# SqueezeAILab/SqueezeLLM

Hardware: AMD Instinct MI355X
Metric: LLaMA-7B-shaped quantised-linear decode throughput (batch 1, all QuantLinearLUT matvecs of the model per token) (higher is better)
Workload: dtype f32; 1 GPU; llama-7b w4 s0 (dense-only), batch=1 decode, 32 layers x 7 linears, op vecquant4matmul_nuq_perchannel; config_name=7b-w4-s0, launch=graph, linears sharing an input (q/k/v, gate/up) fused into one launch each, parallelism=single GPU, world_size=1, rccl_ranks=0

## Files before the change

### squeezellm_amd/csrc/sqllm_kernels.hip

```cpp
#include "sqllm_fused.h"
#include "sqllm_split_common.h"

namespace sqllm {

bool (*g_fused_variant)(int bits, const LaunchArgs& a, hipStream_t stream, hipError_t* err) = nullptr;

constexpr int kXtStride = 36;
constexpr int mfma_codebook_floats(int bits) { return bits == 4 ? 2 * 4096 / 4 : 4 * 8 * 128 / 4; }
constexpr int mfma_lds_floats(int bits, int mb, int waves) {
  return mfma_codebook_floats(bits) + cmax(waves * 16 * mb * kXtStride, waves * 16 * 64);
}

template <int BITS, int MB, int WAVES>
__device__ __forceinline__ void dense_role_mfma(const float* __restrict__ x, const u32x4* __restrict__ q,
                                                float* __restrict__ y, const float* __restrict__ lut, int K, int N,
                                                int batch, int m0, int bid, int n_col_tiles, int units_total,
                                                int units_per_wg, int units_stride, float* lds) {
  using F = Fmt<BITS>;
  constexpr int L = F::kLut, R = F::kRows, KU = F::kK;
  constexpr int NPH = KU / 8;
  constexpr int TR = 16 * MB;
  constexpr int XL = TR / 8;
  constexpr int ESTRIDE = (BITS == 4) ? 256 : 128;
  constexpr int SUBB = (BITS == 4) ? (L * ESTRIDE) / 2 : L * ESTRIDE;
  __builtin_amdgcn_s_waitcnt(0);
  const int tid = threadIdx.x;
  const int lane = tid & 63;
  const int wave = __builtin_amdgcn_readfirstlane(tid >> 6);
  const int i16 = lane & 15, grp = lane >> 4;
  if constexpr ((SQLLM_MFMA_VAR & 64) != 0) {
    const int pr = (wave >> 2) + ((SQLLM_MFMA_VAR & 128) ? 2 * ((bid >> 8) & 1) : 0);
    if (pr == 1) __builtin_amdgcn_s_setprio(1);
    else if (pr == 2) __builtin_amdgcn_s_setprio(2);
    else if (pr == 3) __builtin_amdgcn_s_setprio(3);
  }
  constexpr int kCb = mfma_codebook_floats(BITS);
  float* slabs = lds + kCb;
  float* xt = lds + kCb + wave * (TR * kXtStride);
  constexpr int EPW = 32 / WAVES, RPW = 16 / WAVES;
  constexpr int NE = (BITS == 4) ? EPW : RPW;
  const int st_j = (BITS == 4) ? 2 * (wave & 1) + (lane >> 5) : (wave & 3);
  const int st_h = (BITS == 4) ? (wave >> 1) : (wave >> 2);
  const int row_stride = N / 4;
  const char* qbase = reinterpret_cast<const char*>(q);
  const uint32_t row_bytes = 16u * (uint32_t)row_stride;
  int xrow[XL];
#pragma unroll
  for (int j = 0; j < XL; ++j) {
    int r = m0 + (lane >> 3) + 8 * j;
    if (r > batch - 1) r = batch - 1;
    xrow[j] = r * K + 4 * (lane & 1);
  }
  const int xkq = (lane >> 1) & 3;
  const uint32_t lane_off = 4 * (i16 + 16 * (grp & 1));
  uint32_t tb[4];
#pragma unroll
  for (int j = 0; j < 4; ++j) tb[j] = j * SUBB + 4 * (i16 + 16 * (grp & 1));
  float* xt_w = xt + (lane >> 3) * kXtStride + 8 * xkq + 4 * (lane & 1);
  const float* xt_r = xt + i16 * kXtStride + 8 * grp;

  const unsigned total = (unsigned)n_col_tiles * (unsigned)units_stride;
  unsigned gpos = (unsigned)bid * (unsigned)units_per_wg;
  unsigned gend = gpos + (unsigned)units_per_wg;
  if (gend > total) gend = total;
  while (gpos < gend) {
  const int ct = (int)(gpos / (unsigned)units_stride);
  const int u_beg = (int)(gpos - (unsigned)ct * (unsigned)units_stride);
  if (u_beg >= units_total) { gpos = (unsigned)(ct + 1) * (unsigned)units_stride; continue; }
  int u_end = units_total;
  if ((unsigned)(u_end - u_beg) > gend - gpos) u_end = u_beg + (int)(gend - gpos);
  gpos += (unsigned)(u_end - u_beg);
  if (u_end == units_total) gpos = (unsigned)(ct + 1) * (unsigned)units_stride;
  const int col0 = ct * kTileN;

  float ev[NE];
  {
    int c = col0 + 4 * i16 + st_j;
    if (c > N - 1) c = N - 1;
    const float* src = lut + (size_t)c * L;
    if constexpr (BITS == 4) {
#pragma unroll
      for (int i = 0; i < EPW / 4; ++i) {
        const f32x4 t = *reinterpret_cast<const f32x4*>(src + st_h * EPW + 4 * i);
        ev[4 * i] = t.x; ev[4 * i + 1] = t.y; ev[4 * i + 2] = t.z; ev[4 * i + 3] = t.w;
      }
    } else {
#pragma unroll
      for (int i = 0; i < RPW; ++i) ev[i] = src[2 * (st_h * RPW + i) + (lane >> 5)];
    }
  }
  const int n_groups_wg = (u_end - u_beg + 3) / 4;
  const int n_g = n_groups_wg > wave ? (n_groups_wg - wave + WAVES - 1) / WAVES : 0;
  int cidx = col0 / 4 + i16;
  if (cidx > row_stride - 1) cidx = row_stride - 1;
  const uint32_t lane_bytes = 16u * (uint32_t)cidx;
  auto group_unit = [&](int g, int kq) {
    return u_beg + 4 * (wave + WAVES * g) + kq;
  };
  auto load_w = [&](int g, u32x4 (&dw)[R]) {
    int u = group_unit(g, grp);
    if (u > u_end - 1) u = u_end - 1;
    if (u < u_beg) u = u_beg;
    if (SQLLM_MFMA_VAR & 32) u = u_beg + grp;
    const uint32_t off = (uint32_t)(u * R) * row_bytes + lane_bytes;
#pragma unroll
    for (int r = 0; r < R; ++r) dw[r] = __builtin_nontemporal_load(reinterpret_cast<const u32x4*>(qbase + (off + r * row_bytes)));
  };
  auto load_x = [&](int g, int ph, f32x4 (&dx)[XL]) {
    int u = group_unit(g, xkq);
    if (u > u_end - 1) u = u_end - 1;
    if (u < u_beg) u = u_beg;
    if ((SQLLM_MFMA_VAR & 16) && g > 0) return;
#pragma unroll
    for (int j = 0; j < XL; ++j) dx[j] = *reinterpret_cast<const f32x4*>(x + xrow[j] + u * KU + 8 * ph);
  };
  u32x4 wa[R], wb[R];
  f32x4 xa[XL], xb[XL];
  load_w(0, wa);
  load_x(0, 0, xa);
  asm volatile("" ::: "memory");
  __builtin_amdgcn_sched_barrier(0);
  if constexpr (BITS == 4) {
    float* dst = lds + ((wave & 1) * 4096 + st_h * EPW * ESTRIDE) / 4 + lane;
#pragma unroll
    for (int i = 0; i < EPW; ++i) dst[i * (ESTRIDE / 4)] = ev[i];
  } else {
    float* dst = lds + (st_j * SUBB) / 4 + (lane >> 5) * (ESTRIDE / 4) + (lane & 31);
#pragma unroll
    for (int i = 0; i < RPW; ++i) dst[2 * (st_h * RPW + i) * (ESTRIDE / 4)] = ev[i];
  }
  f32x4 acc[MB][4];
#pragma unroll
  for (int mb = 0; mb < MB; ++mb)
#pragma unroll
    for (int j = 0; j < 4; ++j) acc[mb][j] = f32x4{0.f, 0.f, 0.f, 0.f};
  __syncthreads();

  auto phase = [&](const float (&v)[4][8], const f32x4 (&dx)[XL], int g) {
    const bool live = group_unit(g, xkq) < u_end;
#pragma unroll
    for (int j = 0; j < XL; ++j)
      if (!(SQLLM_MFMA_VAR & 8)) *reinterpret_cast<f32x4*>(xt_w + 8 * j * kXtStride) = live ? dx[j] : f32x4{0.f, 0.f, 0.f, 0.f};
    f32x4 alo[MB], ahi[MB];
#pragma unroll
    for (int mb = 0; mb < MB; ++mb) {
      if constexpr (SQLLM_MFMA_VAR & 8) {
        alo[mb] = dx[0];
        ahi[mb] = dx[XL - 1];
      } else {
        alo[mb] = *reinterpret_cast<const f32x4*>(xt_r + 16 * mb * kXtStride);
        ahi[mb] = *reinterpret_cast<const f32x4*>(xt_r + 16 * mb * kXtStride + 4);
      }
    }
    if (SQLLM_MFMA_VAR & 1) __builtin_amdgcn_s_setprio(1);
#pragma unroll
    for (int s2 = 0; s2 < 8; ++s2)
#pragma unroll
      for (int mb = 0; mb < MB; ++mb) {
        const float a = s2 < 4 ? alo[mb][s2 & 3] : ahi[mb][s2 & 3];
#pragma unroll
        for (int j = 0; j < 4; ++j) {
#if SQLLM_MFMA_FAKE
          acc[mb][j].x = __builtin_fmaf(a, v[j][s2], acc[mb][j].x);
#else
          acc[mb][j] = __builtin_amdgcn_mfma_f32_16x16x4f32(a, v[j][s2], acc[mb][j], 0, 0, 0);
#endif
        }
      }
    if (SQLLM_MFMA_VAR & 1) __builtin_amdgcn_s_setprio(0);
  };
  auto lookups = [&](const u32x4 (&t)[R], auto ph_tag, float (&v)[4][8]) {
    constexpr int PH = decltype(ph_tag)::value;
    if constexpr (SQLLM_MFMA_VAR & 4) {
#pragma unroll
      for (int j = 0; j < 4; ++j)
#pragma unroll
        for (int i = 0; i < 8; ++i) v[j][i] = __builtin_bit_cast(float, t[0].x ^ (uint32_t)(j * 8 + i));
      return;
    }
    if constexpr (BITS == 4) {
      const uint32_t w4[4] = {t[0].x, t[0].y, t[0].z, t[0].w};
#pragma unroll
      for (int j = 0; j < 4; ++j) {
        const uint32_t lo = w4[j] & 0x0F0F0F0Fu, hi = (w4[j] >> 4) & 0x0F0F0F0Fu;
        const int off = (j >> 1) * 4096 + (j & 1) * 128;
        v[j][0] = lds_read_f32(__builtin_amdgcn_perm(lo, lane_off, 0x0C0C0400u) + off);
        v[j][1] = lds_read_f32(__builtin_amdgcn_perm(hi, lane_off, 0x0C0C0400u) + off);
        v[j][2] = lds_read_f32(__builtin_amdgcn_perm(lo, lane_off, 0x0C0C0500u) + off);
        v[j][3] = lds_read_f32(__builtin_amdgcn_perm(hi, lane_off, 0x0C0C0500u) + off);
        v[j][4] = lds_read_f32(__builtin_amdgcn_perm(lo, lane_off, 0x0C0C0600u) + off);
        v[j][5] = lds_read_f32(__builtin_amdgcn_perm(hi, lane_off, 0x0C0C0600u) + off);
        v[j][6] = lds_read_f32(__builtin_amdgcn_perm(lo, lane_off, 0x0C0C0700u) + off);
        v[j][7] = lds_read_f32(__builtin_amdgcn_perm(hi, lane_off, 0x0C0C0700u) + off);
      }
    } else {
      const uint32_t t0[4] = {t[0].x, t[0].y, t[0].z, t[0].w};
      const uint32_t t1[4] = {t[1].x, t[1].y, t[1].z, t[1].w};
      const uint32_t t2[4] = {t[2].x, t[2].y, t[2].z, t[2].w};
#pragma unroll
      for (int j = 0; j < 4; ++j) {
        v[j][0] = lds_read_f32(tb[j] | field3_x128<8 * PH + 0>(t0[j], t1[j], t2[j]));
        v[j][1] = lds_read_f32(tb[j] | field3_x128<8 * PH + 1>(t0[j], t1[j], t2[j]));
        v[j][2] = lds_read_f32(tb[j] | field3_x128<8 * PH + 2>(t0[j], t1[j], t2[j]));
        v[j][3] = lds_read_f32(tb[j] | field3_x128<8 * PH + 3>(t0[j], t1[j], t2[j]));
        v[j][4] = lds_read_f32(tb[j] | field3_x128<8 * PH + 4>(t0[j], t1[j], t2[j]));
        v[j][5] = lds_read_f32(tb[j] | field3_x128<8 * PH + 5>(t0[j], t1[j], t2[j]));
        v[j][6] = lds_read_f32(tb[j] | field3_x128<8 * PH + 6>(t0[j], t1[j], t2[j]));
        v[j][7] = lds_read_f32(tb[j] | field3_x128<8 * PH + 7>(t0[j], t1[j], t2[j]));
      }
    }
  };
  using P0 = std::integral_constant<int, 0>;
  using P1 = std::integral_constant<int, 1>;
  using P2 = std::integral_constant<int, 2>;
  using P3 = std::integral_constant<int, 3>;
  auto decode_group = [&](int g, const u32x4 (&w)[R], f32x4 (&xcur)[XL], u32x4 (&wn)[R], f32x4 (&xn)[XL]) {
    load_w(g + 1, wn);
    float v[4][8];
    if constexpr (NPH == 1) {
      load_x(g + 1, 0, xn);
      if (!(SQLLM_MFMA_VAR & 2)) __builtin_amdgcn_sched_barrier(0);
      lookups(w, P0{}, v);
      phase(v, xcur, g);
    } else {
      f32x4 xo[XL];
      load_x(g, 1, xo);
      if (!(SQLLM_MFMA_VAR & 2)) __builtin_amdgcn_sched_barrier(0);
      lookups(w, P0{}, v);
      phase(v, xcur, g);
      load_x(g, 2, xcur);
      if (!(SQLLM_MFMA_VAR & 2)) __builtin_amdgcn_sched_barrier(0);
      lookups(w, P1{}, v);
      phase(v, xo, g);
      load_x(g, 3, xo);
      if (!(SQLLM_MFMA_VAR & 2)) __builtin_amdgcn_sched_barrier(0);
      lookups(w, P2{}, v);
      phase(v, xcur, g);
      load_x(g + 1, 0, xn);
      if (!(SQLLM_MFMA_VAR & 2)) __builtin_amdgcn_sched_barrier(0);
      lookups(w, P3{}, v);
      phase(v, xo, g);
    }
    if (!(SQLLM_MFMA_VAR & 2)) __builtin_amdgcn_sched_barrier(0);
  };
  for (int g = 0; g < n_g; g += 2) {
    decode_group(g, wa, xa, wb, xb);
    decode_group(g + 1, wb, xb, wa, xa);
  }

  __syncthreads();
  float* slab = slabs + wave * (16 * 64) + (4 * grp) * 64 + 4 * i16;
#pragma unroll
  for (int mb = 0; mb < MB; ++mb) {
    if (mb) __syncthreads();
    *reinterpret_cast<f32x4*>(slab + 0 * 64) = f32x4{acc[mb][0].x, acc[mb][1].x, acc[mb][2].x, acc[mb][3].x};
    *reinterpret_cast<f32x4*>(slab + 1 * 64) = f32x4{acc[mb][0].y, acc[mb][1].y, acc[mb][2].y, acc[mb][3].y};
    *reinterpret_cast<f32x4*>(slab + 2 * 64) = f32x4{acc[mb][0].z, acc[mb][1].z, acc[mb][2].z, acc[mb][3].z};
    *reinterpret_cast<f32x4*>(slab + 3 * 64) = f32x4{acc[mb][0].w, acc[mb][1].w, acc[mb][2].w, acc[mb][3].w};
    __syncthreads();
#pragma unroll
    for (int e = tid; e < 16 * 64; e += WAVES * 64) {
      const int r = m0 + 16 * mb + (e >> 6);
      const int col = col0 + (e & 63);
      float sum = 0.f;
#pragma unroll
      for (int w = 0; w < WAVES; ++w) sum += slabs[w * (16 * 64) + e];
      if (r < batch && col < N) acc_add(y + (size_t)r * N + col, sum);
    }
  }
  }
}

template <int BITS, int MB, int WAVES>
__global__ void __launch_bounds__(WAVES * 64, (BITS == 4 && MB <= 2 && !(SQLLM_MFMA_VAR & 256)) ? 4 : 1)
sqllm_fused_batched(const float* x, const GroupArgs ga) {
  __shared__ __attribute__((aligned(16))) float lds[mfma_lds_floats(BITS, MB, WAVES)];
  const Segment sg = ga.seg[0];
  asm volatile("" ::SQLLM_SEG_OPERANDS(sg), "s"(x));
  __builtin_amdgcn_sched_barrier(0);
  const KernelGeom& gm = sg.gm;
  const int m0 = blockIdx.y * 16 * MB;
  dense_role_mfma<BITS, MB, WAVES>(x, reinterpret_cast<const u32x4*>(sg.q), sg.y, sg.lut, gm.K, gm.N, gm.batch, m0,
                                   (int)blockIdx.x, gm.col_tiles, gm.units_total, gm.units_per_wg, units_stride_of(gm), lds);
}

template <int WAVES>
__global__ void __launch_bounds__(WAVES * 64)
sqllm_sparse_batched(const float* x, const GroupArgs ga, const float* xT, int Bp, int pass_rows) {
  constexpr int T = WAVES * 64;
  __shared__ __attribute__((aligned(16))) float lds[kWideSparseLdsFloats];
  const Segment sg = ga.seg[0];
  asm volatile("" ::SQLLM_SEG_OPERANDS(sg), "s"(x));
  __builtin_amdgcn_sched_barrier(0);
  const KernelGeom& gm = sg.gm;
  const int sp = blockIdx.x;
  const int m0 = blockIdx.y * pass_rows;
  int rows_here = gm.batch - m0;
  if (rows_here > pass_rows) rows_here = pass_rows;
  if (sp < gm.csr_blocks) {
    if (xT) {
      csr_role<T, 1, float, float, true>(x, sg.y, sg.rows, sg.cols, sg.vals, gm.nnz, gm.K, gm.N, m0, rows_here, sp, lds, nullptr, 0, xT, Bp, SQLLM_PROBE_PTR(sg));
    } else {
      constexpr int CBT = 32;
      for (int bb = 0; bb < rows_here; bb += CBT) {
        if (bb) __syncthreads();
        csr_role<T, CBT, float, float>(x, sg.y, sg.rows, sg.cols, sg.vals, gm.nnz, gm.K, gm.N, m0 + bb,
                                       rows_here - bb < CBT ? rows_here - bb : CBT, sp, lds, nullptr, 0);
      }
    }
  } else if (sp < gm.csr_blocks + gm.topx_blocks) {
    for (int bb = 0; bb < rows_here; bb += 64) {
      if (bb) __syncthreads();
      topx_role<T, float, float, false, NoGate, 8>(x, sg.y, sg.full_rows, sg.full_idx, gm.topX, gm.K, gm.N, m0 + bb, rows_here - bb < 64 ? rows_here - bb : 64,
                                 sp - gm.csr_blocks, lds);
    }
  }
}

typedef float f32x8 __attribute__((ext_vector_type(8)));
constexpr int cols_table_floats(int bits) { return bits == 4 ? 17 * 64 : 65 * 64 * 2; }
constexpr int cols_lds_floats(int bits, int bt, int waves) {
  return cmax(cols_table_floats(bits) + waves * bt * 64, cmax(2 * kCsrSpanMax, kTopxLds));
}
constexpr int cols_stage_k(int bt) { return bt * 8 <= 32 ? 8 : 4; }

__device__ __forceinline__ uint32_t field6_x512(uint32_t t0, uint32_t t1, uint32_t t2, int M) {
  const int bit = 6 * M, w = bit >> 5, o = bit & 31;
  const uint32_t lo = (w == 0) ? t0 : (w == 1) ? t1 : t2;
  uint32_t f;
  if (o <= 26) {
    if (o > 9) f = lo >> (o - 9);
    else if (o < 9) f = lo << (9 - o);
    else f = lo;
  } else {
    const uint32_t hi = (w == 0) ? t1 : t2;
    f = __builtin_amdgcn_alignbit(hi, lo, o) << 9;
  }
  return f & 0x7E00u;
}

typedef const __attribute__((address_space(4))) float* cfloatp;
typedef const __attribute__((address_space(4))) char* ccharp;
template <int ST> struct XVec;
template <> struct XVec<4> {
  typedef f32x4 type;
  static __device__ __forceinline__ type load(ccharp base, uint32_t off) {
    return *reinterpret_cast<const __attribute__((address_space(4))) type*>(base + off);
  }
};
template <> struct XVec<8> {
  typedef f32x8 type;
  static __device__ __forceinline__ type load(ccharp base, uint32_t off) {
    return *reinterpret_cast<const __attribute__((address_space(4))) type*>(base + off);
  }
};

template <int BITS, int BT, int WAVES>
__device__ __forceinline__ void dense_role_cols(const float* __restrict__ x, const uint32_t* __restrict__ q,
                                                float* __restrict__ y, const float* __restrict__ lut, int K, int N,
                                                int b0, int nb, int bid, int n_col_tiles, int units_total,
                                                int units_per_wg, int units_stride, float* lds) {
  using F = Fmt<BITS>;
  constexpr int L = F::kLut, R = F::kRows, KU = F::kK;
  constexpr int ST = cols_stage_k(BT);
  constexpr int SPU = KU / ST;
  constexpr int D = BITS == 4 ? 4 : 2;
  constexpr int NB = 2;
  constexpr int NS = D * SPU;
  constexpr int NP = ST / 2;
  constexpr int NA = BT >= 4 ? 1 : 4 / BT;
  using XV = typename XVec<ST>::type;
  static_assert(NS % 2 == 0, "stages alternate between two register sets");
  static_assert(WAVES == 8, "table build assumes 8 waves");
  __builtin_amdgcn_s_waitcnt(0);
  const int tid = threadIdx.x, lane = tid & 63;
  const int w = __builtin_amdgcn_readfirstlane(tid >> 6);
  char* table = reinterpret_cast<char*>(lds);
  float* slabs = lds + cols_table_floats(BITS);
  const uint32_t lane_base = BITS == 4 ? (4u * lane) | 0x1000u : 8u * lane;
  const uint32_t row_bytes = 4u * (uint32_t)N;
  ccharp xrow[BT];
#pragma unroll
  for (int b = 0; b < BT; ++b) xrow[b] = reinterpret_cast<ccharp>(reinterpret_cast<uintptr_t>(x + (size_t)(b0 + (b < nb ? b : nb - 1)) * K));
  uint32_t soff[D][R];
#pragma unroll
  for (int j = 0; j < D; ++j)
#pragma unroll
    for (int r = 0; r < R; ++r) soff[j][r] = (uint32_t)(j * WAVES * R + r) * row_bytes;
  if constexpr (BITS == 4) { if (tid < 64) *reinterpret_cast<float*>(table + 16 * 256 + 4 * tid) = 0.f; }
  else { if (tid < 64) *reinterpret_cast<f32x2*>(table + 64 * 512 + 8 * tid) = f32x2{0.f, 0.f}; }

  const unsigned total = (unsigned)n_col_tiles * (unsigned)units_stride;
  unsigned gpos = (unsigned)bid * (unsigned)units_per_wg;
  unsigned gend = gpos + (unsigned)units_per_wg;
  if (gend > total) gend = total;
  bool first = true;
  while (gpos < gend) {
    const int ct = __builtin_amdgcn_readfirstlane((int)(gpos / (unsigned)units_stride));
    const int u0 = (int)(gpos - (unsigned)ct * (unsigned)units_stride);
    if (u0 >= units_total) { gpos = (unsigned)(ct + 1) * (unsigned)units_stride; continue; }
    int u1 = units_total;
    if ((unsigned)(u1 - u0) > gend - gpos) u1 = u0 + (int)(gend - gpos);
    gpos += (unsigned)(u1 - u0);
    if (u1 == units_total) gpos = (unsigned)(ct + 1) * (unsigned)units_stride;
    const int col0 = ct * kTileN;
    const int col = col0 + lane;
    const int colc = col < N ? col : N - 1;
    const float* lp = lut + (size_t)colc * L;
    float tv[8];
    float thi = 0.f;
    if constexpr (BITS == 4) {
      const f32x2 t = *reinterpret_cast<const f32x2*>(lp + 2 * w);
      tv[0] = t.x; tv[1] = t.y;
    } else {
      const f32x4 ta = *reinterpret_cast<const f32x4*>(lp), tb2 = *reinterpret_cast<const f32x4*>(lp + 4);
      tv[0] = ta.x; tv[1] = ta.y; tv[2] = ta.z; tv[3] = ta.w; tv[4] = tb2.x; tv[5] = tb2.y; tv[6] = tb2.z; tv[7] = tb2.w;
      thi = lp[w];
    }
    const int n_units = u1 - u0;
    const int n_w = n_units > w ? (n_units - w + WAVES - 1) / WAVES : 0;
    const int nc = (n_w + D - 1) / D;
    const __amdgpu_buffer_rsrc_t qrsrc =
        __builtin_amdgcn_make_buffer_rsrc(const_cast<uint32_t*>(q), 0, (uint32_t)(u1 * R) * row_bytes, 0x00020000);
    uint32_t voff[NB];
#pragma unroll
    for (int k = 0; k < NB; ++k) voff[k] = 4u * (uint32_t)colc + (uint32_t)((u0 + w + k * D * WAVES) * R) * row_bytes;
    auto load_chunk = [&](int k, uint32_t (&dst)[D][R]) {
#pragma unroll
      for (int j = 0; j < D; ++j)
#pragma unroll
        for (int r = 0; r < R; ++r) dst[j][r] = __builtin_amdgcn_raw_buffer_load_b32(qrsrc, voff[k], soff[j][r], 2 );
      voff[k] += (uint32_t)(NB * D * WAVES * R) * row_bytes;
    };
    uint32_t wbuf[NB][D][R];
#pragma unroll
    for (int k = 0; k < NB; ++k) load_chunk(k, wbuf[k]);
    asm volatile("" ::: "memory");
    __builtin_amdgcn_sched_barrier(0);
    if (!first) __syncthreads();
    first = false;
    if constexpr (BITS == 4) {
      *reinterpret_cast<float*>(table + (2 * w) * 256 + 4 * lane) = tv[0];
      *reinterpret_cast<float*>(table + (2 * w + 1) * 256 + 4 * lane) = tv[1];
    } else {
#pragma unroll
      for (int i0 = 0; i0 < 8; ++i0) *reinterpret_cast<f32x2*>(table + (8 * w + i0) * 512 + lane_base) = f32x2{tv[i0], thi};
    }
    __syncthreads();

    f32x2 acc[BT][NA];
#pragma unroll
    for (int b = 0; b < BT; ++b)
#pragma unroll
      for (int a = 0; a < NA; ++a) acc[b][a] = f32x2{0.f, 0.f};
    struct St { f32x2 v[NP]; XV x[BT]; };
    auto issue = [&](const uint32_t (&buf)[D][R], int st, int cc, St& o) {
      const int j = st / SPU, sub = st % SPU;
      const int i = cc * D + j;
      const bool live = i < n_w;
      if constexpr (BITS == 4) {
        const uint32_t lo = buf[j][0] & 0x0F0F0F0Fu, hi = (buf[j][0] >> 4) & 0x0F0F0F0Fu;
#define SQ_L(WORD, SEL) *reinterpret_cast<const float __attribute__((address_space(3)))*>(__builtin_amdgcn_perm(WORD, lane_base, SEL))
#pragma unroll
        for (int m = 0; m < NP; ++m) {
          const uint32_t sel = live ? 0x0C0C0400u + ((uint32_t)(sub * NP + m) << 8) : 0x0C0C0100u;
          o.v[m] = f32x2{SQ_L(lo, sel), SQ_L(hi, sel)};
        }
#undef SQ_L
      } else {
        const uint32_t lane_or_dead = lane_base | (live ? 0u : 0x8000u);
#pragma unroll
        for (int m = 0; m < NP; ++m)
          o.v[m] = *reinterpret_cast<const f32x2 __attribute__((address_space(3)))*>(
              lane_or_dead | field6_x512(buf[j][0], buf[j][1], buf[j][2], sub * NP + m));
      }
      int u = u0 + w + i * WAVES;
      if (u > u1 - 1) u = u1 - 1;
      uint32_t koff = 4u * (uint32_t)(u * KU + sub * ST);
      asm volatile("" : "+s"(koff));
#pragma unroll
      for (int b = 0; b < BT; ++b) o.x[b] = XVec<ST>::load(xrow[b], koff);
    };
    auto fmas = [&](const St& o) {
#pragma unroll
      for (int m = 0; m < NP; ++m)
#pragma unroll
        for (int b = 0; b < BT; ++b)
          acc[b][m % NA] = __builtin_elementwise_fma(o.v[m], f32x2{o.x[b][2 * m], o.x[b][2 * m + 1]}, acc[b][m % NA]);
    };
    St sa, sb;
    issue(wbuf[0], 0, 0, sa);
    __builtin_amdgcn_sched_barrier(0);
    for (int c = 0; c < nc; c += NB) {
#pragma unroll
      for (int k = 0; k < NB; ++k) {
#pragma unroll
        for (int st = 0; st < NS; st += 2) {
          __builtin_amdgcn_s_waitcnt(0xC07F);
          issue(wbuf[k], st + 1, c + k, sb);
          __builtin_amdgcn_sched_barrier(0);
          fmas(sa);
          __builtin_amdgcn_sched_barrier(0);
          __builtin_amdgcn_s_waitcnt(0xC07F);
          if (st + 2 < NS) issue(wbuf[k], st + 2, c + k, sa);
          else issue(wbuf[(k + 1) % NB], 0, c + k + 1, sa);
          __builtin_amdgcn_sched_barrier(0);
          fmas(sb);
          __builtin_amdgcn_sched_barrier(0);
        }
        load_chunk(k, wbuf[k]);
        __builtin_amdgcn_sched_barrier(0);
      }
    }

#pragma unroll
    for (int b = 0; b < BT; ++b) {
      f32x2 t = acc[b][0];
#pragma unroll
      for (int a = 1; a < NA; ++a) t += acc[b][a];
      slabs[(w * BT + b) * 64 + lane] = t.x + t.y;
    }
    __syncthreads();
    for (int e = tid; e < BT * 64; e += WAVES * 64) {
      const int b = e >> 6, c = e & 63;
      float sum = 0.f;
#pragma unroll
      for (int ww = 0; ww < WAVES; ++ww) sum += slabs[(ww * BT + b) * 64 + c];
      if (b < nb && col0 + c < N) acc_add(y + (size_t)(b0 + b) * N + col0 + c, sum);
    }
  }
}

template <int BITS, int BT, int WAVES>
__global__ void __launch_bounds__(WAVES * 64)
sqllm_fused_cols(const float* x, const GroupArgs ga) {
  constexpr int T = WAVES * 64;
  __shared__ __attribute__((aligned(16))) float lds[cols_lds_floats(BITS, BT, WAVES)];
  Segment sg = ga.seg[0];
  const int n_seg = ga.n_seg, blk1 = ga.block0[1], blk2 = ga.block0[2], blk3 = ga.block0[3];
  asm volatile("" ::SQLLM_SEG_OPERANDS(sg), "s"(x), "s"(n_seg), "s"(blk1), "s"(blk2), "s"(blk3));
  __builtin_amdgcn_sched_barrier(0);
  int bid = blockIdx.x;
  int s = 0;
  if (n_seg > 1 && bid >= blk1) s = 1;
  if (n_seg > 2 && bid >= blk2) s = 2;
  if (n_seg > 3 && bid >= blk3) s = 3;
  if (s != 0) {
    sg = ga.seg[s];
    asm volatile("" ::SQLLM_SEG_OPERANDS(sg));
    bid -= s == 1 ? blk1 : s == 2 ? blk2 : blk3;
  }
  const KernelGeom& gm = sg.gm;
  const int b0 = blockIdx.y * BT;
  int nb = gm.batch - b0;
  if (nb > BT) nb = BT;
  const int d = bid - gm.dense_block0;
  const int sp = bid < gm.dense_block0 ? bid : -1;
  if (d >= 0 && d < gm.dense_blocks) {
    dense_role_cols<BITS, BT, WAVES>(x, sg.q, sg.y, sg.lut, gm.K, gm.N, b0, nb, d, gm.col_tiles, gm.units_total,
                                     gm.units_per_wg,
                                     gm.dense_blocks == gm.col_tiles * gm.k_slices ? gm.k_slices * gm.units_per_wg : gm.units_total, lds);
  } else if (sp >= 0 && sp < gm.csr_blocks) {
    csr_role<T, BT, float, float>(x, sg.y, sg.rows, sg.cols, sg.vals, gm.nnz, gm.K, gm.N, b0, nb, sp, lds, nullptr, 0);
  } else if (sp >= gm.csr_blocks && sp < gm.csr_blocks + gm.topx_blocks) {
    topx_role<T, float, float, false, NoGate, (BT < 4 ? BT : 4)>(x, sg.y, sg.full_rows, sg.full_idx, gm.topX, gm.K, gm.N, b0, nb, sp - gm.csr_blocks, lds);
  }
}

template <int BITS, bool LIN>
static hipError_t launch_bt(const LaunchArgs& a, hipStream_t stream) {
  const int batch = a.ga.seg[0].gm.batch;
  if constexpr (!LIN) {
    switch (batch_tile_op(batch)) {
      case 3: return launch_inst<BITS, 3, kWaves, 0, LIN>(a, stream);
      case 5: return launch_inst<BITS, 5, kWaves, 0, LIN>(a, stream);
      case 6: return launch_inst<BITS, 6, kWaves, 0, LIN>(a, stream);
      case 7: return launch_inst<BITS, 7, kWaves, 0, LIN>(a, stream);
      default: break;
    }
  }
  if constexpr (BITS == 4 && !LIN) {
    if (batch == 1) {
      bool brief = true;
      for (int i = 0; i < a.ga.n_seg; ++i) brief = brief && a.ga.seg[i].gm.units_per_wg <= 2 * kWaves * 4;
      if (brief) return launch_inst<BITS, 1, kWaves, 0, LIN, true>(a, stream);
    }
  }
  switch (batch_tile(batch)) {
    case 1: return launch_inst<BITS, 1, kWaves, 0, LIN>(a, stream);
    case 2: return launch_inst<BITS, 2, kWaves, 0, LIN>(a, stream);
    case 4: return launch_inst<BITS, 4, kWaves, 0, LIN>(a, stream);
    default: return launch_inst<BITS, 8, kWaves, 0, LIN>(a, stream);
  }
}

template <int BITS, int MB>
static hipError_t launch_mfma_inst(const LaunchArgs& a, hipStream_t stream) {
  const KernelGeom& gm = a.ga.seg[0].gm;
  dim3 grid(gm.dense_blocks, (gm.batch + 16 * MB - 1) / (16 * MB));
  auto kern = sqllm_fused_batched<BITS, MB, kWaves>;
  const float* x = static_cast<const float*>(a.x);
  return launch_kernel(kern, grid, dim3(kWaves * 64), 0, stream, a.ev_start, a.ev_stop, x, a.ga);
}

template <int BITS>
static hipError_t launch_mfma_bits(const LaunchArgs& a, hipStream_t stream) {
  return with_row_blocks(mfma_row_blocks(a.ga.seg[0].gm.batch), [&](auto mb) { return launch_mfma_inst<BITS, decltype(mb)::value>(a, stream); });
}

template <int BITS, int BT>
static hipError_t launch_cols_inst(const LaunchArgs& a, hipStream_t stream) {
  const KernelGeom& gm = a.ga.seg[0].gm;
  dim3 grid(a.ga.block0[a.ga.n_seg], (gm.batch + BT - 1) / BT);
  auto kern = sqllm_fused_cols<BITS, BT, kWaves>;
  const float* x = static_cast<const float*>(a.x);
  return launch_kernel(kern, grid, dim3(kWaves * 64), 0, stream, a.ev_start, a.ev_stop, x, a.ga);
}

template <int BITS>
static hipError_t launch_cols_bits(const LaunchArgs& a, hipStream_t stream) {
  switch (batch_tile_op(a.ga.seg[0].gm.batch)) {
    case 1: return launch_cols_inst<BITS, 1>(a, stream);
    case 2: return launch_cols_inst<BITS, 2>(a, stream);
    case 3: return launch_cols_inst<BITS, 3>(a, stream);
    case 4: return launch_cols_inst<BITS, 4>(a, stream);
    case 5: return launch_cols_inst<BITS, 5>(a, stream);
    case 6: return launch_cols_inst<BITS, 6>(a, stream);
    case 7: return launch_cols_inst<BITS, 7>(a, stream);
    default: return launch_cols_inst<BITS, 8>(a, stream);
  }
}

hipError_t launch_batched_cols(int bits, const LaunchArgs& a, hipStream_t stream) {
  return bits == 4 ? launch_cols_bits<4>(a, stream) : launch_cols_bits<3>(a, stream);
}

hipError_t launch_batched_sparse(const LaunchArgs& a, hipStream_t stream) {
  const KernelGeom& gm = a.ga.seg[0].gm;
  if (gm.csr_blocks + gm.topx_blocks <= 0) return hipSuccess;
  const int blocks = gm.csr_blocks + gm.topx_blocks;
  const int pass_rows = (long long)blocks * ((gm.batch + kSparsePassRows - 1) / kSparsePassRows) >= 2048 ? kSparsePassRows : 64;
  dim3 grid(blocks, (gm.batch + pass_rows - 1) / pass_rows);
  auto kern = sqllm_sparse_batched<kWaves>;
  const float* x = static_cast<const float*>(a.x);
  return launch_kernel(kern, grid, dim3(kWaves * 64), 0, stream, a.ev_start, a.ev_stop, x, a.ga, a.xT, a.Bp, pass_rows);
}

hipError_t launch_batched_mfma(int bits, const LaunchArgs& a, hipStream_t stream) {
  return bits == 4 ? launch_mfma_bits<4>(a, stream) : launch_mfma_bits<3>(a, stream);
}

__global__ void __launch_bounds__(256) sqllm_transpose_vec(const float* __restrict__ x, float* __restrict__ xT, int batch, int K, int Bp) {
  __shared__ float tile[64][65];
  const int k0 = blockIdx.x * 64, r0 = blockIdx.y * 64;
  const int tx = threadIdx.x & 63, ty = threadIdx.x >> 6;
#pragma unroll
  for (int i = 0; i < 16; ++i) {
    const int r = r0 + ty + 4 * i, k = k0 + tx;
    tile[ty + 4 * i][tx] = (r < batch && k < K) ? x[(size_t)r * K + k] : 0.f;
  }
  __syncthreads();
#pragma unroll
  for (int i = 0; i < 16; ++i) {
    const int k = k0 + ty + 4 * i, r = r0 + tx;
    if (k < K) xT[(size_t)k * Bp + r] = tile[tx][ty + 4 * i];
  }
}

__global__ void __launch_bounds__(256) sqllm_transpose_small(const float* __restrict__ x, float* __restrict__ xT, int batch, int K, int lr) {
  const unsigned t = blockIdx.x * 256u + threadIdx.x;
  const unsigned rp = 1u << lr;
  const unsigned b = t & (rp - 1u);
  const unsigned k = (t >> lr) * 4u;
  if (k >= (unsigned)K) return;
  f32x4 v = {0.f, 0.f, 0.f, 0.f};
  if (b < (unsigned)batch) v = *reinterpret_cast<const f32x4*>(x + (size_t)b * K + k);
  float* dst = xT + ((size_t)k << lr) + b;
  dst[0] = v.x;
  dst[rp] = v.y;
  dst[2 * rp] = v.z;
  dst[3 * rp] = v.w;
}

__global__ void __launch_bounds__(256) sqllm_prepare_small(const float* __restrict__ x, float* __restrict__ xT, u32x4* __restrict__ planes,
                                                           int batch, int K, int lr) {
  const unsigned t = blockIdx.x * 256u + threadIdx.x;
  const unsigned b = t & 15u;
  const unsigned k8 = t >> 4;
  const unsigned k = 8u * k8;
  if (k >= (unsigned)K + 32u) return;
  float v[8] = {0.f, 0.f, 0.f, 0.f, 0.f, 0.f, 0.f, 0.f};
  if (k < (unsigned)K && b < (unsigned)batch) {
    const f32x4 a = *reinterpret_cast<const f32x4*>(x + (size_t)b * K + k), c = *reinterpret_cast<const f32x4*>(x + (size_t)b * K + k + 4);
    v[0] = a.x; v[1] = a.y; v[2] = a.z; v[3] = a.w; v[4] = c.x; v[5] = c.y; v[6] = c.z; v[7] = c.w;
  }
  uint32_t h[4], m[4], l[4];
  split8(v, h, m, l);
  u32x4* dst = planes + ((size_t)(k8 >> 2) * 3u * 64u + 16u * (k8 & 3u) + b);
  dst[0] = u32x4{h[0], h[1], h[2], h[3]};
  dst[64] = u32x4{m[0], m[1], m[2], m[3]};
  dst[128] = u32x4{l[0], l[1], l[2], l[3]};
  const unsigned rp = 1u << lr;
  if (xT && k < (unsigned)K && b < rp) {
    float* d = xT + ((size_t)k << lr) + b;
#pragma unroll
    for (int j = 0; j < 8; ++j) d[(size_t)j << lr] = v[j];
  }
}

hipError_t prepare_small(const float* x, float* xT, void* planes, int batch, int K, hipStream_t stream, hipEvent_t ev_start) {
  const unsigned threads = (unsigned)(K / 8 + 4) * 16u;
  const dim3 grid((threads + 255u) / 256u);
  return launch_kernel(sqllm_prepare_small, grid, dim3(256), 0, stream, ev_start, nullptr, x, xT, static_cast<u32x4*>(planes), batch, K,
                       small_rows_log2(batch));
}

hipError_t transpose_small(const float* x, float* xT, int batch, int K, hipStream_t stream, hipEvent_t ev_start) {
  const int lr = small_rows_log2(batch);
  const unsigned threads = (unsigned)(K / 4) << lr;
  const dim3 grid((threads + 255u) / 256u);
  return launch_kernel(sqllm_transpose_small, grid, dim3(256), 0, stream, ev_start, nullptr, x, xT, batch, K, lr);
}

hipError_t transpose_vec(const float* x, float* xT, int batch, int K, int Bp, hipStream_t stream, hipEvent_t ev_start) {
  return launch_kernel(sqllm_transpose_vec, dim3((K + 63) / 64, Bp / 64), dim3(256), 0, stream, ev_start, nullptr, x, xT, batch, K, Bp);
}

__global__ void sqllm_check_csr(const int* __restrict__ rows, int N, int nnz, int* flag) {
  const int i = blockIdx.x * blockDim.x + threadIdx.x;
  if (i == 0 && (rows[0] != 0 || rows[N] != nnz)) atomicOr(flag, 1);
  if (i < N && rows[i + 1] < rows[i]) atomicOr(flag, 2);
}

hipError_t check_csr(const int* rows, int N, int nnz, hipStream_t stream, int* bad) {
  *bad = 0;
  hipStreamCaptureStatus cs = hipStreamCaptureStatusNone;
  if (hipStreamIsCapturing(stream, &cs) == hipSuccess && cs != hipStreamCaptureStatusNone) return hipSuccess;
  int* flag = nullptr;
  hipError_t e;
  if ((e = hipMallocAsync(reinterpret_cast<void**>(&flag), sizeof(int), stream)) != hipSuccess) return e;
  if ((e = hipMemsetAsync(flag, 0, sizeof(int), stream)) == hipSuccess) {
    hipLaunchKernelGGL(sqllm_check_csr, dim3((N + 255) / 256), dim3(256), 0, stream, rows, N, nnz, flag);
    e = hipGetLastError();
  }
  if (e == hipSuccess) e = hipMemcpyAsync(bad, flag, sizeof(int), hipMemcpyDeviceToHost, stream);
  (void)hipFreeAsync(flag, stream);
  if (e != hipSuccess) return e;
  return hipStreamSynchronize(stream);
}

hipError_t launch_fused(int bits, const LaunchArgs& a, hipStream_t stream) {
  if (g_fused_variant) {
    hipError_t err = hipSuccess;
    if (g_fused_variant(bits, a, stream, &err)) return err;
  }
  if (a.linear) return bits == 4 ? launch_bt<4, true>(a, stream) : launch_bt<3, true>(a, stream);
  return bits == 4 ? launch_bt<4, false>(a, stream) : launch_bt<3, false>(a, stream);
}

}
```

Baseline: 805.0 tokens/s.

## Add batch-1 software pipeline with grouped activation loads and byte-perm LUT lookups

For batch size 1, the inner loop is restructured. Activation vectors are loaded in groups into two alternating SGPR sets, one group ahead, while codebook lookups run one step ahead with finer-grained waitcnt values. For 4-bit weights, nibbles are extracted with v_perm to build LDS addresses directly. A guard-free path is used for full chunks and the bounds check is kept only for the tail. The aim is to hide scalar load latency and cut per-step address arithmetic, at the cost of code size, register pressure and more fragile hand-tuned waitcnt logic.

```diff
diff --git a/squeezellm_amd/csrc/sqllm_kernels.hip b/squeezellm_amd/csrc/sqllm_kernels.hip
--- a/squeezellm_amd/csrc/sqllm_kernels.hip
+++ b/squeezellm_amd/csrc/sqllm_kernels.hip
@@ -488,6 +488,87 @@
         for (int b = 0; b < BT; ++b)
           acc[b][m % NA] = __builtin_elementwise_fma(o.v[m], f32x2{o.x[b][2 * m], o.x[b][2 * m + 1]}, acc[b][m % NA]);
     };
+    if constexpr (BT == 1) {
+      constexpr int GS = 32 / ST;
+      constexpr int LPS = BITS == 4 ? 2 * NP : NP;
+      static_assert(NS % GS == 0 && (NB * NS / GS) % 2 == 0, "vec groups alternate between two SGPR sets");
+      struct V { f32x2 v[NP]; };
+      XV xs[2][GS];
+      auto look = [&](const uint32_t (&buf)[D][R], int st, int cc, V& o, auto guard) {
+        const int j = st / SPU, sub = st % SPU;
+        bool live = true;
+        if constexpr (decltype(guard)::value) live = cc * D + j < n_w;
+        if constexpr (BITS == 4) {
+          const uint32_t lo = buf[j][0] & 0x0F0F0F0Fu, hi = (buf[j][0] >> 4) & 0x0F0F0F0Fu;
+#define SQ_L(WORD, SEL) *reinterpret_cast<const float __attribute__((address_space(3)))*>(__builtin_amdgcn_perm(WORD, lane_base, SEL))
+#pragma unroll
+          for (int m = 0; m < NP; ++m) {
+            const uint32_t sel = live ? 0x0C0C0400u + ((uint32_t)(sub * NP + m) << 8) : 0x0C0C0100u;
+            o.v[m] = f32x2{SQ_L(lo, sel), SQ_L(hi, sel)};
+          }
+#undef SQ_L
+        } else {
+          const uint32_t lane_or_dead = lane_base | (live ? 0u : 0x8000u);
+#pragma unroll
+          for (int m = 0; m < NP; ++m)
+            o.v[m] = *reinterpret_cast<const f32x2 __attribute__((address_space(3)))*>(
+                lane_or_dead | field6_x512(buf[j][0], buf[j][1], buf[j][2], sub * NP + m));
+        }
+      };
+      auto vec_group = [&](int st0, int cc, XV (&xg)[GS]) {
+#pragma unroll
+        for (int g = 0; g < GS; ++g) {
+          const int j = (st0 + g) / SPU, sub = (st0 + g) % SPU;
+          int u = u0 + w + (cc * D + j) * WAVES;
+          if (u > u1 - 1) u = u1 - 1;
+          uint32_t koff = 4u * (uint32_t)(u * KU + sub * ST);
+          asm volatile("" : "+s"(koff));
+          xg[g] = XVec<ST>::load(xrow[0], koff);
+        }
+      };
+      auto fma1 = [&](const V& o, const XV& xv) {
+#pragma unroll
+        for (int m = 0; m < NP; ++m)
+          acc[0][m % NA] = __builtin_elementwise_fma(o.v[m], f32x2{xv[2 * m], xv[2 * m + 1]}, acc[0][m % NA]);
+      };
+      V va, vb;
+      auto chunk_pair = [&](int c, auto guard) {
+#pragma unroll
+        for (int k = 0; k < NB; ++k) {
+#pragma unroll
+          for (int st = 0; st < NS; ++st) {
+            V& cur = (st & 1) ? vb : va;
+            V& nxt = (st & 1) ? va : vb;
+            const int set = ((k * NS + st) / GS) & 1, pos = st % GS;
+            const bool wrap = st + 1 == NS;
+            if (pos == GS - 1) __builtin_amdgcn_s_waitcnt(0xC07F);
+            if (wrap) look(wbuf[(k + 1) % NB], 0, c + k + 1, nxt, guard);
+            else look(wbuf[k], st + 1, c + k, nxt, guard);
+            __builtin_amdgcn_sched_barrier(0);
+            if (pos != GS - 1) {
+              __builtin_amdgcn_s_waitcnt(0xC07F | (LPS << 8));
+              if (pos == GS - 2) {
+                __builtin_amdgcn_sched_barrier(0);
+                if (st + 2 == NS) vec_group(0, c + k + 1, xs[set ^ 1]);
+                else vec_group(st + 2, c + k, xs[set ^ 1]);
+              }
+              __builtin_amdgcn_sched_barrier(0);
+            }
+            fma1(cur, xs[set][pos]);
+            __builtin_amdgcn_sched_barrier(0);
+          }
+          load_chunk(k, wbuf[k]);
+          __builtin_amdgcn_sched_barrier(0);
+        }
+      };
+      vec_group(0, 0, xs[0]);
+      __builtin_amdgcn_s_waitcnt(0xC07F);
+      look(wbuf[0], 0, 0, va, std::true_type{});
+      __builtin_amdgcn_sched_barrier(0);
+      int c = 0;
+      for (; (c + NB) * D <= n_w; c += NB) chunk_pair(c, std::false_type{});
+      for (; c < nc; c += NB) chunk_pair(c, std::true_type{});
+    } else {
     St sa, sb;
     issue(wbuf[0], 0, 0, sa);
     __builtin_amdgcn_sched_barrier(0);
@@ -511,6 +592,7 @@
         load_chunk(k, wbuf[k]);
         __builtin_amdgcn_sched_barrier(0);
       }
+    }
     }
 
 #pragma unroll
```

New measurement: 820.1 tokens/s, median of 6. +1.9%, better.
